# icsharpcode/SharpZipLib

Hardware: NVIDIA B200
Metric: DEFLATE level-6 compress + inflate GB/s (uncompressed) at 1/2/4/8 B200 vs C# ref (higher is better)
Workload: dtype u8

## Files before the change

### include/b200z.h

```cpp
#ifndef B200Z_H
#define B200Z_H
#include <stdint.h>
#ifdef __cplusplus
extern "C" {
#endif

typedef enum b200z_status {
	B200Z_OK = 0,
	B200Z_E_ARG = 1,
	B200Z_E_STATE = 2,
	B200Z_E_DATA = 3,
	B200Z_E_INTERNAL = 4,
	B200Z_E_CUDA = 5,
	B200Z_E_UNSUPPORTED = 6,
	B200Z_E_NOMEM = 7,
	B200Z_E_NEED_INPUT = 8
} b200z_status;

enum { B200Z_WRAP_RAW = 0, B200Z_WRAP_ZLIB = 1, B200Z_WRAP_GZIP = 2, B200Z_WRAP_RAW_CRC32 = 3  };
enum { B200Z_STRATEGY_DEFAULT = 0, B200Z_STRATEGY_FILTERED = 1, B200Z_STRATEGY_HUFFMAN_ONLY = 2 };
enum {
	B200Z_END_FINISH = 0,
	B200Z_END_FLUSH_FINISH = 1,
	B200Z_END_FLUSH = 2
};

const char *b200z_last_error(void);
int b200z_version(void);
int b200z_init(int device);
int b200z_static_tables_size(void);
int b200z_static_tables_export(uint8_t *blob, int32_t cap);
int b200z_static_tables_import(const uint8_t *blob, int32_t len);
int b200z_static_tables_broadcast(void *nccl_comm, int32_t root, int32_t rank, void *cuda_stream);

int b200z_crc32(const uint8_t *buf, int64_t len, uint32_t *value);
int b200z_adler32(const uint8_t *buf, int64_t len, uint32_t *value);
int b200z_checksum_batch_device(int kind, const uint8_t *d_data, const int64_t *off, const int64_t *len, int32_t n,
                                uint32_t *d_value, void *cuda_stream);

typedef struct b200z_plan b200z_plan;

#define B200Z_HIST_NONE 0
#define B200Z_HIST_DICTIONARY 1
#define B200Z_HIST_CONTINUE 2
typedef struct b200z_history {
	int32_t kind;
	int32_t check_seeded;
	const int64_t *hist_len;
	const int64_t *pos_base;
	const int32_t *bit_base;
	const uint8_t *const *hist_mask;
	const int32_t *chunk_count;
	const int64_t *const *chunk_len;
	const int32_t *undrained_last;
	void *const *engine_state;
	struct b200z_stored_state *stored_state;
} b200z_history;
typedef struct b200z_stored_state {
	int32_t strstart, block_start;
	uint32_t slides, input_off;
} b200z_stored_state;
int64_t b200z_engine_state_bytes(void);
int b200z_deflate_plan_create_ex(int32_t n, const int64_t *in_len, int level, int strategy, int wrap, int end_mode,
                                 const b200z_history *hist, b200z_plan **plan);

int b200z_deflate_plan_create(int32_t n, const int64_t *in_len, int level, int strategy, int wrap, int end_mode,
                              b200z_plan **plan);
int b200z_inflate_plan_create(int32_t n, const int64_t *comp_len, const int64_t *out_cap, int wrap, b200z_plan **plan);
int b200z_inflate_plan_create_ex(int32_t n, const int64_t *comp_len, const int64_t *out_cap, int wrap,
                                 const int64_t *dict_len, b200z_plan **plan);
int b200z_inflate_plan_set_start_bits(b200z_plan *plan, const int32_t *start_bit);
int b200z_inflate_plan_set_lengths(b200z_plan *plan, const int64_t *comp_len, const int64_t *dict_len);
int b200z_plan_get_restart_points(b200z_plan *plan, int64_t *bit, int64_t *out_pos, void *cuda_stream);
int b200z_plan_get_stats(b200z_plan *plan, uint32_t *v, int32_t cap, void *cuda_stream);
int b200z_plan_destroy(b200z_plan *plan);
int64_t b200z_plan_in_bytes(const b200z_plan *plan);
int64_t b200z_plan_out_bytes(const b200z_plan *plan);
int64_t b200z_plan_in_offset(const b200z_plan *plan, int32_t i);
int64_t b200z_plan_data_offset(const b200z_plan *plan, int32_t i);
int64_t b200z_plan_out_offset(const b200z_plan *plan, int32_t i);
int64_t b200z_plan_out_capacity(const b200z_plan *plan, int32_t i);
int64_t b200z_plan_workspace_bytes(const b200z_plan *plan);
int32_t b200z_plan_launches(const b200z_plan *plan);
int b200z_plan_set_timing(b200z_plan *plan, int enable);
int b200z_plan_get_timings(b200z_plan *plan, char *names, int32_t names_cap, float *ms, int32_t cap, int32_t *count);
int b200z_plan_run(b200z_plan *plan, const uint8_t *d_in, uint8_t *d_out, int64_t *d_out_len, int32_t *d_status,
                   uint32_t *d_check, int64_t *d_in_used, void *cuda_stream);
#define B200Z_STAGE_SEARCH 1
#define B200Z_STAGE_ENCODE 2
int b200z_plan_run_stages(b200z_plan *plan, const uint8_t *d_in, uint8_t *d_out, int64_t *d_out_len, int32_t *d_status,
                          uint32_t *d_check, int64_t *d_in_used, int stages, void *cuda_stream);

int b200z_plan_pack(b200z_plan *plan, const uint8_t *d_out, const int64_t *d_out_len, uint8_t *d_packed,
                    int64_t *d_packed_off, void *cuda_stream);

typedef struct b200z_pipeline b200z_pipeline;
int b200z_deflate_pipeline_create(int32_t n, const int64_t *in_len, int level, int strategy, int wrap, int end_mode, int depth,
                                  b200z_pipeline **pipe);
int b200z_inflate_pipeline_create(int32_t n, const int64_t *comp_len, const int64_t *out_cap, int wrap, int depth,
                                  b200z_pipeline **pipe);
int b200z_pipeline_submit(b200z_pipeline *pipe, const uint8_t *const *in);
int b200z_pipeline_collect(b200z_pipeline *pipe, uint8_t *const *out, const int64_t *out_cap, int64_t *out_len, int64_t *in_used,
                           uint32_t *check, int32_t *status);
int32_t b200z_pipeline_in_flight(const b200z_pipeline *pipe);
int b200z_pipeline_destroy(b200z_pipeline *pipe);

int b200z_deflate_batch(const uint8_t *const *in, const int64_t *in_len, int32_t n, int level, int strategy, int wrap,
                        int end_mode, uint8_t *const *out, const int64_t *out_cap, int64_t *out_len, uint32_t *check,
                        int32_t *status);
int b200z_inflate_batch(const uint8_t *const *in, const int64_t *in_len, int32_t n, int wrap, uint8_t *const *out,
                        const int64_t *out_cap, int64_t *out_len, int64_t *in_used, uint32_t *check, int32_t *status);
int b200z_release_cached(void);

int b200z_device_count(void);
int b200z_partition_by_bytes(const int64_t *len, int32_t n, int32_t parts, int32_t *first);
int b200z_deflate_batch_multi(const int32_t *devices, int32_t n_devices, const uint8_t *const *in, const int64_t *in_len, int32_t n,
                              int level, int strategy, int wrap, int end_mode, uint8_t *const *out, const int64_t *out_cap,
                              int64_t *out_len, uint32_t *check, int32_t *status);
int b200z_inflate_batch_multi(const int32_t *devices, int32_t n_devices, const uint8_t *const *in, const int64_t *in_len, int32_t n,
                              int wrap, uint8_t *const *out, const int64_t *out_cap, int64_t *out_len, int64_t *in_used,
                              uint32_t *check, int32_t *status);
int64_t b200z_deflate_bound(int64_t len);

int b200z_deflater_create(int level, int raw , void **h);
int b200z_deflater_destroy(void *h);
int b200z_deflater_reset(void *h);
int b200z_deflater_set_level(void *h, int level);
// ... 52 lines not shown
```

### sharpziplib_b200/_lib.py

```python
import ctypes as C
import os

_HERE = os.path.dirname(os.path.abspath(__file__))
SO_PATH = os.path.join(_HERE, "libb200z.so")

OK, E_ARG, E_STATE, E_DATA, E_INTERNAL, E_CUDA, E_UNSUPPORTED, E_NOMEM, E_NEED_INPUT = range(9)
WRAP_RAW, WRAP_ZLIB, WRAP_GZIP, WRAP_RAW_CRC32 = 0, 1, 2, 3
END_FINISH, END_FLUSH_FINISH, END_FLUSH = 0, 1, 2


class SharpZipBaseException(Exception):
    """Mirror of ICSharpCode.SharpZipLib.SharpZipBaseException (Core/Exceptions/SharpZipBaseException.cs)."""


class StreamDecodingException(SharpZipBaseException):
    pass


class B200zUnsupported(NotImplementedError):
    """A call sequence this build does not accelerate (never emulated on the CPU)."""


class B200zCudaError(RuntimeError):
    pass


class InvalidOperationException(RuntimeError):
    pass


def raise_for(rc):
    if rc == OK:
        return
    msg = lib().b200z_last_error().decode("utf-8", "replace")
    code = rc & 0xFF
    if code == E_ARG:
        raise ValueError(msg)
    if code == E_STATE:
        raise InvalidOperationException(msg)
    if code == E_DATA:
        raise SharpZipBaseException(msg)
    if code == E_UNSUPPORTED:
        raise B200zUnsupported(msg)
    if code == E_CUDA:
        raise B200zCudaError(msg)
    if code == E_NOMEM:
        raise MemoryError(msg)
    if code == E_NEED_INPUT:
        raise SharpZipBaseException("Unexpected EOF")
    raise RuntimeError("b200z status %d: %s" % (rc, msg))


_lib = None

_SIGS = {
    "b200z_last_error": (C.c_char_p, []),
    "b200z_version": (C.c_int, []),
    "b200z_init": (C.c_int, [C.c_int]),
    "b200z_static_tables_size": (C.c_int, []),
    "b200z_static_tables_export": (C.c_int, [C.c_void_p, C.c_int32]),
    "b200z_static_tables_import": (C.c_int, [C.c_void_p, C.c_int32]),
    "b200z_crc32": (C.c_int, [C.c_void_p, C.c_int64, C.POINTER(C.c_uint32)]),
    "b200z_adler32": (C.c_int, [C.c_void_p, C.c_int64, C.POINTER(C.c_uint32)]),
    "b200z_checksum_batch_device": (C.c_int, [C.c_int, C.c_void_p, C.c_void_p, C.c_void_p, C.c_int32, C.c_void_p, C.c_void_p]),
    "b200z_deflate_plan_create": (C.c_int, [C.c_int32, C.c_void_p, C.c_int, C.c_int, C.c_int, C.c_int, C.POINTER(C.c_void_p)]),
    "b200z_deflate_plan_create_ex": (C.c_int, [C.c_int32, C.c_void_p, C.c_int, C.c_int, C.c_int, C.c_int, C.c_void_p,
                                               C.POINTER(C.c_void_p)]),
    "b200z_inflate_plan_create": (C.c_int, [C.c_int32, C.c_void_p, C.c_void_p, C.c_int, C.POINTER(C.c_void_p)]),
    "b200z_inflate_plan_create_ex": (C.c_int, [C.c_int32, C.c_void_p, C.c_void_p, C.c_int, C.c_void_p, C.POINTER(C.c_void_p)]),
    "b200z_inflate_plan_set_start_bits": (C.c_int, [C.c_void_p, C.c_void_p]),
    "b200z_plan_get_restart_points": (C.c_int, [C.c_void_p, C.c_void_p, C.c_void_p, C.c_void_p]),
    "b200z_inflate_plan_set_lengths": (C.c_int, [C.c_void_p, C.c_void_p, C.c_void_p]),
    "b200z_plan_get_stats": (C.c_int, [C.c_void_p, C.c_void_p, C.c_int32, C.c_void_p]),
    "b200z_plan_data_offset": (C.c_int64, [C.c_void_p, C.c_int32]),
    "b200z_plan_destroy": (C.c_int, [C.c_void_p]),
    "b200z_plan_in_bytes": (C.c_int64, [C.c_void_p]),
    "b200z_plan_out_bytes": (C.c_int64, [C.c_void_p]),
    "b200z_plan_in_offset": (C.c_int64, [C.c_void_p, C.c_int32]),
    "b200z_plan_out_offset": (C.c_int64, [C.c_void_p, C.c_int32]),
    "b200z_plan_out_capacity": (C.c_int64, [C.c_void_p, C.c_int32]),
    "b200z_plan_workspace_bytes": (C.c_int64, [C.c_void_p]),
    "b200z_plan_launches": (C.c_int32, [C.c_void_p]),
    "b200z_plan_set_timing": (C.c_int, [C.c_void_p, C.c_int]),
    "b200z_plan_get_timings": (C.c_int, [C.c_void_p, C.c_char_p, C.c_int32, C.c_void_p, C.c_int32, C.POINTER(C.c_int32)]),
    "b200z_plan_pack": (C.c_int, [C.c_void_p, C.c_void_p, C.c_void_p, C.c_void_p, C.c_void_p, C.c_void_p]),
    "b200z_plan_run": (C.c_int, [C.c_void_p, C.c_void_p, C.c_void_p, C.c_void_p, C.c_void_p, C.c_void_p, C.c_void_p, C.c_void_p]),
    "b200z_plan_run_stages": (C.c_int, [C.c_void_p, C.c_void_p, C.c_void_p, C.c_void_p, C.c_void_p, C.c_void_p, C.c_void_p, C.c_int,
                                        C.c_void_p]),
    "b200z_deflate_batch": (C.c_int, [C.c_void_p, C.c_void_p, C.c_int32, C.c_int, C.c_int, C.c_int, C.c_int, C.c_void_p, C.c_void_p, C.c_void_p, C.c_void_p, C.c_void_p]),
    "b200z_inflate_batch": (C.c_int, [C.c_void_p, C.c_void_p, C.c_int32, C.c_int, C.c_void_p, C.c_void_p, C.c_void_p, C.c_void_p, C.c_void_p, C.c_void_p]),
    "b200z_release_cached": (C.c_int, []),
    "b200z_device_count": (C.c_int, []),
    "b200z_static_tables_broadcast": (C.c_int, [C.c_void_p, C.c_int32, C.c_int32, C.c_void_p]),
    "b200z_aes_derive_keys": (C.c_int, [C.c_void_p, C.c_void_p, C.c_void_p, C.c_int32, C.c_int32, C.c_void_p]),
    "b200z_aes_state_bytes": (C.c_int64, []),
    "b200z_aes_device": (C.c_int, [C.c_void_p, C.c_void_p, C.c_void_p, C.c_void_p, C.c_int64, C.c_int32, C.c_int32, C.c_void_p, C.c_int32,
                                   C.c_void_p, C.c_int32, C.c_void_p, C.c_void_p]),
    "b200z_aes_batch": (C.c_int, [C.c_void_p, C.c_void_p, C.c_int32, C.c_int32, C.c_void_p, C.c_int32, C.c_void_p, C.c_void_p]),
    "b200z_aes_transform_create": (C.c_int, [C.c_void_p, C.c_int32, C.c_void_p, C.c_int32, C.c_int32, C.POINTER(C.c_void_p)]),
    "b200z_aes_transform_block": (C.c_int, [C.c_void_p, C.c_void_p, C.c_int64, C.c_void_p]),
    "b200z_aes_transform_pwd_verifier": (C.c_int, [C.c_void_p, C.c_void_p]),
    "b200z_aes_transform_auth_code": (C.c_int, [C.c_void_p, C.c_void_p]),
    "b200z_aes_transform_destroy": (C.c_int, [C.c_void_p]),
    "b200z_pkzip_generate_keys": (C.c_int, [C.c_void_p, C.c_int64, C.c_void_p]),
    "b200z_pkzip_device": (C.c_int, [C.c_void_p, C.c_void_p, C.c_void_p, C.c_void_p, C.c_int32, C.c_void_p, C.c_int32, C.c_void_p]),
    "b200z_pkzip_batch": (C.c_int, [C.c_void_p, C.c_void_p, C.c_int32, C.c_void_p, C.c_int32, C.c_void_p]),
    "b200z_partition_by_bytes": (C.c_int, [C.c_void_p, C.c_int32, C.c_int32, C.c_void_p]),
    "b200z_deflate_batch_multi": (C.c_int, [C.c_void_p, C.c_int32, C.c_void_p, C.c_void_p, C.c_int32, C.c_int, C.c_int, C.c_int, C.c_int, C.c_void_p, C.c_void_p, C.c_void_p, C.c_void_p, C.c_void_p]),
    "b200z_inflate_batch_multi": (C.c_int, [C.c_void_p, C.c_int32, C.c_void_p, C.c_void_p, C.c_int32, C.c_int, C.c_void_p, C.c_void_p, C.c_void_p, C.c_void_p, C.c_void_p, C.c_void_p]),
    "b200z_deflate_pipeline_create": (C.c_int, [C.c_int32, C.c_void_p, C.c_int, C.c_int, C.c_int, C.c_int, C.c_int, C.POINTER(C.c_void_p)]),
    "b200z_inflate_pipeline_create": (C.c_int, [C.c_int32, C.c_void_p, C.c_void_p, C.c_int, C.c_int, C.POINTER(C.c_void_p)]),
    "b200z_pipeline_submit": (C.c_int, [C.c_void_p, C.c_void_p]),
    "b200z_pipeline_collect": (C.c_int, [C.c_void_p, C.c_void_p, C.c_void_p, C.c_void_p, C.c_void_p, C.c_void_p, C.c_void_p]),
    "b200z_pipeline_in_flight": (C.c_int32, [C.c_void_p]),
    "b200z_pipeline_destroy": (C.c_int, [C.c_void_p]),
    "b200z_deflate_bound": (C.c_int64, [C.c_int64]),
    "b200z_engine_state_bytes": (C.c_int64, []),
    "b200z_deflater_create": (C.c_int, [C.c_int, C.c_int, C.POINTER(C.c_void_p)]),
    "b200z_deflater_destroy": (C.c_int, [C.c_void_p]),
    "b200z_deflater_reset": (C.c_int, [C.c_void_p]),
    "b200z_deflater_set_level": (C.c_int, [C.c_void_p, C.c_int]),
    "b200z_deflater_get_level": (C.c_int, [C.c_void_p, C.POINTER(C.c_int)]),
    "b200z_deflater_set_strategy": (C.c_int, [C.c_void_p, C.c_int]),
    "b200z_deflater_set_dictionary": (C.c_int, [C.c_void_p, C.c_void_p, C.c_int32]),
    "b200z_deflater_set_input": (C.c_int, [C.c_void_p, C.c_void_p, C.c_int32]),
    "b200z_deflater_flush": (C.c_int, [C.c_void_p]),
# ... 54 lines not shown
```

### sharpziplib_b200/csrc/b200z_api.cu

```cuda
#include <algorithm>
#include <cstdarg>
#include <cstdio>
#include <cstring>
#include <functional>
#include <mutex>
#include <thread>
#include <utility>

#include "b200z_internal.cuh"
#include <dlfcn.h>

namespace b200z {

static thread_local std::string g_err;
static std::mutex g_mu;
static thread_local int t_device = -1;

void set_error(const char *fmt, ...) {
	char buf[512];
	va_list ap;
	va_start(ap, fmt);
	vsnprintf(buf, sizeof(buf), fmt, ap);
	va_end(ap);
	g_err = buf;
// ... 463 lines not shown
	}
	const int n = plan->n;
	std::vector<int64_t> dl((size_t)n);
	std::vector<uint32_t> d32((size_t)n);
	for (int i = 0; i < n; i++) {
		const int64_t D = dict_len ? dict_len[i] : 0;
		if (comp_len[i] < 0 || comp_len[i] > plan->comp_cap[(size_t)i] || D < 0 || D > plan->dict_cap[(size_t)i]) {
			set_error("stream %d: %lld compressed / %lld dictionary bytes exceed what the plan was created for (%lld / %lld)", i,
			          (long long)comp_len[i], (long long)D, (long long)plan->comp_cap[(size_t)i], (long long)plan->dict_cap[(size_t)i]);
			return B200Z_E_ARG;
		}
		dl[(size_t)i] = comp_len[i];
		d32[(size_t)i] = (uint32_t)D;
	}
	for (int i = 0; i < n; i++) {
		if (!plan->hist.empty()) plan->hist[(size_t)i] = d32[(size_t)i];
		plan->in_off[(size_t)i] = plan->comp_off[(size_t)i] - d32[(size_t)i];
		plan->in_len[(size_t)i] = comp_len[i] + d32[(size_t)i];
	}
	if (n) {
		B200Z_CUDA(cudaMemcpy(plan->ws.at<int64_t>(plan->o_in_len), dl.data(), 8ull * n, cudaMemcpyHostToDevice));
		B200Z_CUDA(cudaMemcpy(plan->ws.at<uint32_t>(plan->o_hist), d32.data(), 4ull * n, cudaMemcpyHostToDevice));
	}
	return B200Z_OK;
}

int b200z_plan_get_restart_points(b200z_plan *plan, int64_t *bit, int64_t *out_pos, void *cuda_stream) {
	DeviceGuard guard(plan ? plan->device : -1);
	if (!plan || plan->kind != 1 || (plan->n > 0 && (!bit || !out_pos))) {
		set_error("bad arguments");
		return B200Z_E_ARG;
	}
	if (plan->n == 0) return B200Z_OK;
	std::vector<int64_t> rp(2 * (size_t)plan->n);
	cudaStream_t s = (cudaStream_t)cuda_stream;
	B200Z_CUDA(cudaMemcpyAsync(rp.data(), plan->ws.at<int64_t>(plan->o_restart), 16ull * plan->n, cudaMemcpyDeviceToHost, s));
	B200Z_CUDA(cudaStreamSynchronize(s));
	for (int i = 0; i < plan->n; i++) {
		bit[i] = rp[2 * (size_t)i];
		out_pos[i] = rp[2 * (size_t)i + 1];
	}
	return B200Z_OK;
}

int b200z_plan_get_stats(b200z_plan *plan, uint32_t *v, int32_t cap, void *cuda_stream) {
	DeviceGuard guard(plan ? plan->device : -1);
	if (!plan || plan->kind != 1 || !v || cap < 0) {
		set_error("bad arguments");
		return B200Z_E_ARG;
	}
	return inflate_plan_stats(plan, v, cap, (cudaStream_t)cuda_stream);
}

int b200z_plan_set_timing(b200z_plan *plan, int enable) {
	if (!plan) return B200Z_E_ARG;
	plan->timing = enable != 0;
	plan->ev_used = 0;
	return B200Z_OK;
}

int b200z_plan_get_timings(b200z_plan *plan, char *names, int32_t names_cap, float *ms, int32_t cap, int32_t *count) {
	DeviceGuard guard(plan ? plan->device : -1);
	if (!plan || !ms || !count) return B200Z_E_ARG;
	*count = 0;
	std::string nm;
	for (int i = 0; i + 1 < plan->ev_used && *count < cap; i++) {
		float t = 0;
		cudaError_t e = cudaEventElapsedTime(&t, plan->ev[i], plan->ev[i + 1]);
		if (e != cudaSuccess) return cuda_fail(e, "cudaEventElapsedTime", __FILE__, __LINE__);
		ms[*count] = t;
		nm += plan->ev_name[i];
		nm += ";";
		++*count;
	}
	if (names && names_cap > 0) {
		strncpy(names, nm.c_str(), (size_t)names_cap - 1);
		names[names_cap - 1] = 0;
	}
	return B200Z_OK;
}

int b200z_plan_destroy(b200z_plan *plan) {
	DeviceGuard guard(plan ? plan->device : -1);
	if (!plan) return B200Z_OK;
	for (cudaEvent_t e : plan->ev) cudaEventDestroy(e);
	plan->ws.release();
	delete plan;
	return B200Z_OK;
}
int64_t b200z_plan_in_bytes(const b200z_plan *p) { return p->in_bytes; }
int64_t b200z_plan_out_bytes(const b200z_plan *p) { return p->out_bytes; }
int64_t b200z_plan_in_offset(const b200z_plan *p, int32_t i) { return p->in_off[i]; }
int64_t b200z_plan_data_offset(const b200z_plan *p, int32_t i) {
	return p->in_off[i] + (p->hist.empty() ? 0 : p->hist[i]);
}
int64_t b200z_plan_out_offset(const b200z_plan *p, int32_t i) { return p->out_off[i]; }
int64_t b200z_plan_out_capacity(const b200z_plan *p, int32_t i) { return p->out_cap[i]; }
int64_t b200z_plan_workspace_bytes(const b200z_plan *p) { return p->ws.size; }
int32_t b200z_plan_launches(const b200z_plan *p) { return p->launches; }

int b200z_plan_run(b200z_plan *plan, const uint8_t *d_in, uint8_t *d_out, int64_t *d_out_len, int32_t *d_status,
                   uint32_t *d_check, int64_t *d_in_used, void *cuda_stream) {
	return b200z_plan_run_stages(plan, d_in, d_out, d_out_len, d_status, d_check, d_in_used, B200Z_STAGE_SEARCH | B200Z_STAGE_ENCODE,
	                             cuda_stream);
}

// ... 1328 lines not shown
```

### sharpziplib_b200/csrc/b200z_deflate.cu

```cuda
#include <cuda_pipeline.h>

#include "b200z_internal.cuh"
#include "b200z_tma.cuh"

namespace b200z {

constexpr int kRun = 65536;
constexpr int kTile = 32768;
constexpr int kTileData = 2 * kTile + 320;
constexpr int kMatchThreads = 1024;
constexpr int kMatchClasses = 16;

__device__ __forceinline__ uint32_t same_hash_mask(uint32_t h, bool valid, int lane) {
	uint32_t eq = __ballot_sync(0xffffffffu, valid);
#pragma unroll
	for (int b = 0; b < 15; b++) {
		const bool bit = (h >> b) & 1u;
		const uint32_t bal = __ballot_sync(0xffffffffu, bit);
		eq &= bit ? bal : ~bal;
	}
	return valid ? eq : (1u << lane);
}

constexpr int kLinkChunk = 512;
constexpr int kLinkProducers = 8;
constexpr int kLinkThreads = 32 * (1 + kLinkProducers);
constexpr int kLinkRebase = 16384;
constexpr int kLinksSmem = 65536 + 2 * kLinkChunk * 4;

__global__ void __launch_bounds__(kLinkThreads) k_links(const uint8_t *__restrict__ in, uint16_t *__restrict__ link,
                                                        const int64_t *__restrict__ in_off, const int64_t *__restrict__ in_len,
                                                        const int2 *__restrict__ run_desc, const uint32_t *__restrict__ hist,
                                                        const uint8_t *__restrict__ hmask, const int64_t *__restrict__ hm_off,
                                                        uint32_t run_len) {
	extern __shared__ __align__(16) uint8_t lsm[];
	uint16_t *head = reinterpret_cast<uint16_t *>(lsm);
	uint32_t *info = reinterpret_cast<uint32_t *>(lsm + 65536);
	const int lane = threadIdx.x & 31, warp = threadIdx.x >> 5;
	const int2 rd = run_desc[blockIdx.x];
	const uint32_t n = (uint32_t)in_len[rd.x];
	const uint8_t *data = in + in_off[rd.x];
	uint16_t *lnk = link + in_off[rd.x];
	const uint32_t start = (uint32_t)rd.y;
	const uint32_t run_end = (n - start > run_len) ? start + run_len : n;
	const uint32_t warm = start >= 32768u ? start - 32768u : 0u;
	const uint32_t H = hist[rd.x];
	const uint8_t *hm = hmask + hm_off[rd.x];
	for (int i = threadIdx.x; i < 16384; i += kLinkThreads) reinterpret_cast<uint32_t *>(head)[i] = 0;
	uint32_t winbase = warm;
	auto produce = [&](uint32_t cb, int which) {
		constexpr int G = kLinkChunk / 32 / kLinkProducers;
		uint32_t hh[G];
		bool vv[G];
#pragma unroll
		for (int j = 0; j < G; j++) {
			const uint32_t p = cb + 32u * (uint32_t)(warp - 1 + kLinkProducers * j) + lane;
			bool valid = p + 2 < n;
			uint32_t h = 0;
			if (p + 2 < n) h = hash3(__ldg(data + p), __ldg(data + p + 1), __ldg(data + p + 2));
			if (p < H && valid) valid = __ldg(hm + p) == 0;
			hh[j] = h;
			vv[j] = valid;
		}
#pragma unroll
// ... 39 lines not shown
				const uint32_t v = head[h];
				const bool valid = (w >> 15) & 1u;
				uint32_t q = v ? winbase + v - 1 : 0xFFFFFFFFu;
				if ((w >> 16) & 1u) q = base + ((w >> 17) & 31u);
				__syncwarp();
				if (valid && ((w >> 22) & 1u)) head[h] = (uint16_t)(p - winbase + 1);
				__syncwarp();
				const uint32_t d = (valid && q != 0xFFFFFFFFu) ? p - q : 0u;
				if (p >= start && p < run_end) lnk[p] = (d <= (uint32_t)kMaxDist) ? (uint16_t)d : (uint16_t)0;
				w = wn;
			}
		} else if (cb + kLinkChunk < run_end) {
			produce(cb + kLinkChunk, which ^ 1);
		}
		__syncthreads();
	}
}

__global__ void __launch_bounds__(kMatchThreads, 1)
    k_match(const uint8_t *__restrict__ in, const uint16_t *__restrict__ link, uint2 *__restrict__ mt,
            const int64_t *__restrict__ in_off, const int64_t *__restrict__ in_len, const int2 *__restrict__ tile_desc,
            const uint32_t *__restrict__ hist, const int64_t *__restrict__ bias, uint32_t *__restrict__ scratch, LevelParams lp) {
	extern __shared__ __align__(16) uint8_t smem[];
	uint8_t *s_data = smem;
	uint16_t *s_link = reinterpret_cast<uint16_t *>(smem + kTileData);
	const int2 td = tile_desc[blockIdx.x];
	const uint32_t n = (uint32_t)in_len[td.x];
	const int64_t off = in_off[td.x];
	const uint8_t *data = in + off;
	const uint16_t *lnk = link + off;
	const uint32_t t0 = (uint32_t)td.y;
	const uint32_t t1 = (n - t0 > (uint32_t)kTile) ? t0 + kTile : n;
	const uint32_t w0 = t0 >= (uint32_t)kTile ? t0 - kTile : 0u;
	uint32_t dend = t1 + 272;
	if (dend > n) dend = n;
	__shared__ BulkBarrier s_bar;
	if (threadIdx.x == 0) bulk_barrier_init(&s_bar);
	__syncthreads();
	{
		const uint32_t nbytes = dend - w0;
		const uint32_t nvec = nbytes >> 4;
		const uint32_t nl = t1 - w0;
		const uint32_t nlv = nl >> 3;
		if (threadIdx.x == 0) {
			bulk_expect(&s_bar, 16u * (nvec + nlv));
			bulk_copy_start(&s_bar, s_data, data + w0, 16u * nvec);
			bulk_copy_start(&s_bar, s_link, lnk + w0, 16u * nlv);
		}
		for (uint32_t i = (nvec << 4) + threadIdx.x; i < nbytes; i += kMatchThreads) s_data[i] = data[w0 + i];
		for (uint32_t i = (nlv << 3) + threadIdx.x; i < nl; i += kMatchThreads) s_link[i] = lnk[w0 + i];
	}
	bulk_wait(&s_bar, 0);
	__syncthreads();
	uint2 *out = mt + off;
	const uint32_t chain = (uint32_t)lp.chain, budgetB = chain >> 2;
	const uint32_t H = hist[td.x];
	const uint32_t ab = (uint32_t)bias[td.x];
	__shared__ uint32_t s_cls[2][kMatchClasses];
	if (threadIdx.x < 2 * kMatchClasses) (&s_cls[0][0])[threadIdx.x] = 0;
	__syncthreads();
	uint16_t *order = reinterpret_cast<uint16_t *>(scratch + off + t0);
	uint32_t cw[4] = {0u, 0u, 0u, 0u};
	const int lane = threadIdx.x & 31;
#pragma unroll
	for (int k = 0; k < kTile / kMatchThreads; k++) {
		const uint32_t p = t0 + threadIdx.x + (uint32_t)k * kMatchThreads;
		uint32_t cls = 0;
		if (p < t1 && p >= H) {
			const uint32_t la = n - p;
			uint32_t d = la >= (uint32_t)kMinMatch ? (uint32_t)s_link[p - w0] : 0u;
			if (d > (uint32_t)kMaxDist - (is_slide_pos(p + ab) ? 1u : 0u)) d = 0;
			if (d == 0) out[p] = make_uint2(0u, 0u);
			else {
				const uint32_t is = p - w0;
				uint32_t dist = d, hops = 1;
				while (hops < 8) {
					const uint32_t l2 = s_link[is - dist];
					if (l2 == 0 || dist + l2 >= (uint32_t)kMaxDist) break;
					dist += l2;
					++hops;
				}
				if (hops < 8) cls = hops <= 1 ? 1u : hops <= 2 ? 2u : hops <= 4 ? 3u : hops <= 6 ? 4u : 5u;
				else {
					uint32_t est = (8u * (uint32_t)kMaxDist) / dist;
					if (est > chain) est = chain;
					cls = est <= 11 ? 6u : est <= 16 ? 7u : est <= 23 ? 8u : est <= 32 ? 9u : est <= 45 ? 10u : est <= 64 ? 11u
					      : est <= 91 ? 12u : est <= 128 ? 13u : est <= 512 ? 14u : 15u;
				}
			}
		}
		const uint32_t peers = __match_any_sync(0xffffffffu, cls);
		if (cls && lane == __ffs((int)peers) - 1) atomicAdd(&s_cls[0][cls], (uint32_t)__popc(peers));
		cw[k >> 3] |= cls << ((k & 7) * 4);
	}
	__syncthreads();
	uint32_t total = 0;
	{
		uint32_t b = 0;
		uint32_t mine = 0;
		for (int c = kMatchClasses - 1; c >= 1; c--) {
			if ((int)threadIdx.x == c) mine = b;
			b += s_cls[0][c];
		}
		total = b;
		__syncthreads();
		if (threadIdx.x >= 1 && threadIdx.x < kMatchClasses) s_cls[1][threadIdx.x] = mine;
		__syncthreads();
	}
#pragma unroll
	for (int k = 0; k < kTile / kMatchThreads; k++) {
		const uint32_t cls = (cw[k >> 3] >> ((k & 7) * 4)) & 15u;
		const uint32_t peers = __match_any_sync(0xffffffffu, cls);
		uint32_t slot = 0;
		const int leader = __ffs((int)peers) - 1;
		if (cls && lane == leader) slot = atomicAdd(&s_cls[1][cls], (uint32_t)__popc(peers));
		slot = __shfl_sync(0xffffffffu, slot, leader);
		if (cls) order[slot + (uint32_t)__popc(peers & ((1u << lane) - 1u))] = (uint16_t)(threadIdx.x + (uint32_t)k * kMatchThreads);
	}
	__syncthreads();
	for (uint32_t i = threadIdx.x; i < total; i += kMatchThreads) {
		const uint32_t p = t0 + (uint32_t)__ldcg(&order[i]);
		uint32_t resA = 0, resB = 0;
		const uint32_t la = n - p;
		const uint32_t d = (uint32_t)s_link[p - w0];
		if (d != 0) {
			const uint32_t maxlen = la < (uint32_t)kMaxMatch ? la : (uint32_t)kMaxMatch;
			const uint32_t nice = la < (uint32_t)lp.nice ? la : (uint32_t)lp.nice;
			const uint32_t is = p - w0;
			const uint8_t *sp = s_data + is;
			uint32_t m = kMinMatch - 1, bd = 0, dist = d, cnt = 0;
			bool haveB = false;
			uint32_t stop = budgetB ? budgetB : chain;
			const uint32_t s0 = sp[0], s1 = sp[1];
			uint32_t scan_end1 = s1, scan_end = sp[2];
			uint32_t sw0, sw1;
			{
				const uint32_t as = is + 2;
				const uint32_t *ws = reinterpret_cast<const uint32_t *>(s_data + (as & ~3u));
				const uint32_t w1 = ws[1], sh = (as & 3u) * 8u;
				sw0 = __funnelshift_r(ws[0], w1, sh);
				sw1 = __funnelshift_r(w1, ws[2], sh);
			}
			for (;;) {
				const uint32_t ic = is - dist;
				const uint8_t *c = s_data + ic;
				++cnt;
				if (c[m] == scan_end && c[m - 1] == scan_end1 && c[0] == s0 && c[1] == s1) {
					uint32_t l = 2;
					if (maxlen >= 10) {
						const uint32_t ac = ic + 2;
						const uint32_t *wc = reinterpret_cast<const uint32_t *>(s_data + (ac & ~3u));
						const uint32_t w1 = wc[1], sh = (ac & 3u) * 8u;
						uint32_t x = __funnelshift_r(wc[0], w1, sh) ^ sw0;
						if (x) {
							l = 2 + ((uint32_t)(__ffs((int)x) - 1) >> 3);
							goto lcp_done;
						}
						x = __funnelshift_r(w1, wc[2], sh) ^ sw1;
						if (x) {
							l = 6 + ((uint32_t)(__ffs((int)x) - 1) >> 3);
							goto lcp_done;
						}
						l = 10;
					}
					while (l + 4 <= maxlen) {
						const uint32_t ac = ic + l, as = is + l;
						const uint32_t *wc = reinterpret_cast<const uint32_t *>(s_data + (ac & ~3u));
						const uint32_t *ws = reinterpret_cast<const uint32_t *>(s_data + (as & ~3u));
						const uint32_t x = __funnelshift_r(wc[0], wc[1], (ac & 3u) * 8u) ^ __funnelshift_r(ws[0], ws[1], (as & 3u) * 8u);
						if (x) {
							l += (uint32_t)(__ffs((int)x) - 1) >> 3;
							goto lcp_done;
						}
						l += 4;
					}
					while (l < maxlen && c[l] == sp[l]) ++l;
				lcp_done:
					if (l > m) {
						m = l;
						bd = dist;
						if (m >= nice) break;
						scan_end1 = sp[m - 1];
						scan_end = sp[m];
					}
				}
				if (cnt == stop) {
					if (stop == chain) break;
					resB = m >= (uint32_t)kMinMatch ? pack_match(m, bd) : 0u;
					haveB = true;
					stop = chain;
				}
				const uint32_t l2 = s_link[is - dist];
				if (l2 == 0) break;
				dist += l2;
				if (dist >= (uint32_t)kMaxDist) break;
			}
			resA = m >= (uint32_t)kMinMatch ? pack_match(m, bd) : 0u;
			if (!haveB) resB = resA;
		}
		out[p] = make_uint2(resA, resB);
	}
}

constexpr int kSegShift = 5;
constexpr int kSeg = 1 << kSegShift;
constexpr int kRound = 32 * kSeg;
constexpr int kParseWarm = 128;
constexpr int kSegStride = kSeg + 2;
constexpr int kParseDatOff = 32 * kSegStride * 8;
constexpr int kParseSmem = kParseDatOff + kRound + 48;

struct ChunkDesc {
	int32_t stream;
	uint32_t c0, c1;
};

__device__ __forceinline__ ParseCarry shfl_carry(const ParseCarry &c, int src) {
	ParseCarry r;
	r.st.p = __shfl_sync(0xffffffffu, c.st.p, src);
	r.st.mlen = __shfl_sync(0xffffffffu, c.st.mlen, src);
	r.st.mstart = __shfl_sync(0xffffffffu, c.st.mstart, src);
	r.st.prevAvail = __shfl_sync(0xffffffffu, c.st.prevAvail, src);
	r.last_top = __shfl_sync(0xffffffffu, c.last_top, src);
	return r;
}

__device__ __forceinline__ ParseCarry clean_carry(uint32_t p) {
	ParseCarry c;
	parse_init(c.st);
	c.st.p = p;
	c.last_top = p;
	return c;
}

struct RoundRec {
	uint32_t p, mlen, mstart, prevAvail, last_top, cnt;
};
__device__ __forceinline__ ParseCarry rec_carry(const RoundRec &r) {
	ParseCarry c;
	c.st.p = r.p;
	c.st.mlen = r.mlen;
	c.st.mstart = r.mstart;
	c.st.prevAvail = r.prevAvail;
	c.last_top = r.last_top;
	return c;
}

__device__ __forceinline__ uint32_t parse_round(uint8_t *smem, const uint8_t *data, const uint16_t *lnk, const uint2 *tab,
                                                uint32_t n, uint32_t H, uint32_t ab, uint32_t base, const LevelParams &lp,
                                                int strategy, ParseCarry &carry, uint32_t *sround) {
	uint2 *s_tab = reinterpret_cast<uint2 *>(smem);
	uint8_t *s_dat = smem + kParseDatOff;
	const int lane = threadIdx.x & 31;
// ... 1252 lines not shown
		    p->fast_head_smem ? nullptr : ws.at<uint16_t>(p->o_fhead), ws.at<uint32_t>(p->o_fcounter));
	} else {
		if (do_search) {
		p->mark(s, "k_links");
		if (p->n_runs) k_links<<<p->n_runs, kLinkThreads, kLinksSmem, s>>>(d_in, link, in_off, in_len, ws.at<int2>(p->o_run_desc), hist,
			                                                         ws.at<uint8_t>(p->o_hmask), ws.at<int64_t>(p->o_hm_off), (uint32_t)p->link_run);
		p->mark(s, "k_match");
		if (p->n_tiles)
			k_match<<<p->n_tiles, kMatchThreads, kTileData + 2 * 2 * kTile, s>>>(d_in, link, mt, in_off, in_len,
			                                                                   ws.at<int2>(p->o_tile_desc), hist, bias, sym, lp);
		}
		if (!do_encode) {
			B200Z_CUDA(cudaGetLastError());
			return B200Z_OK;
		}
		p->mark(s, "k_parse");
		{
			uint32_t *sym_local = ws.at<uint32_t>(p->o_sym_local);
			const uint32_t *rnd_off = ws.at<uint32_t>(p->o_rnd_off);
			RoundRec *recs = ws.at<RoundRec>(p->o_recs);
			uint32_t *rnd_symoff = ws.at<uint32_t>(p->o_rnd_symoff);
			if (p->n_chunks)
				k_parse_chunk<<<p->n_chunks, 32, kParseSmem, s>>>(d_in, link, mt, sym_local, in_off, in_len, ws.at<ChunkDesc>(p->o_chunks),
				                                                 rnd_off, recs, ws.at<RoundRec>(p->o_ents), hist, bias, lp, p->strategy, parse_warm());
			k_parse_fix<<<n, 32, kParseSmem, s>>>(d_in, link, mt, sym_local, in_off, in_len, rnd_off, recs, ws.at<RoundRec>(p->o_ents),
			                                      p->parse_chunk, hist, bias, lp, p->strategy);
			k_parse_scan<<<n, 256, 0, s>>>(d_in, in_off, in_len, rnd_off, recs, rnd_symoff, sym, nsyms, nblocks, blk_off, blk_start,
			                               blk_ptop, hist, p->end_mode);
			if (p->n_rgroups)
				k_parse_gather<<<p->n_rgroups, 128, 0, s>>>(sym_local, sym, in_off, in_len, ws.at<int2>(p->o_rgroups), rnd_off, recs,
				                                           rnd_symoff, blk_off, blk_start, blk_ptop, hist);
		}
	}
	p->mark(s, "k_plan");
	k_plan<<<p->n_blkmax, kPlanThreads, 0, s>>>(sym, in_off, in_len, nsyms, nblocks, blk_off, blk_desc, blk_start, blk_ptop, meta,
	                                   tables, bias, p->end_mode);
	p->mark(s, "k_scan");
	k_scan<<<(n + 127) / 128, 128, 0, s>>>(n, nblocks, blk_off, meta, d_out, out_off, out_cap, d_out_len, d_status,
	                                       d_out_bits, bit_base, p->end_mode);
	p->mark(s, "k_emit");
	k_emit<<<p->n_blkmax, 256, 0, s>>>(d_in, sym, d_out, in_off, out_off, nblocks, blk_off, blk_desc, meta, tables);
	p->mark(s, "checksum");
	if (p->wrap != B200Z_WRAP_RAW && d_check) {
		int rc = checksum_launch(p->wrap == B200Z_WRAP_ZLIB ? 1 : 0, d_in, ws.at<int64_t>(p->o_ck_off), ws.at<int64_t>(p->o_ck_len), n,
		                         ws.at<CkTile>(p->o_ck_desc), p->n_ck_tiles, ws.at<unsigned long long>(p->o_ck_acc), d_check,
		                         ck_fresh, s);
		if (rc) return rc;
	}
	p->mark(s, "end");
	B200Z_CUDA(cudaGetLastError());
	return B200Z_OK;
}

}
```

### sharpziplib_b200/csrc/b200z_internal.cuh

```cuda
#pragma once
#include <cuda_runtime.h>
#include <stdint.h>
#include <string>
#include <vector>

#include "../../include/b200z.h"
#include "b200z_core.cuh"
#include "b200z_crc.cuh"

namespace b200z {

void set_error(const char *fmt, ...);
int cuda_fail(cudaError_t e, const char *what, const char *file, int line);

#define B200Z_CUDA(call)                                                                   \
	do {                                                                                   \
		cudaError_t e__ = (call);                                                          \
		if (e__ != cudaSuccess) return ::b200z::cuda_fail(e__, #call, __FILE__, __LINE__); \
	} while (0)

int ensure_init();
int current_device();

struct DeviceGuard {
// ... 72 lines not shown
	int64_t o_in_off = 0, o_in_len = 0, o_out_off = 0, o_out_cap = 0;
	int64_t o_run_desc = 0, o_tile_desc = 0, o_blk_desc = 0, o_blk_off = 0;
	int64_t o_link = 0, o_mt = 0, o_sym = 0, o_nsyms = 0, o_nblocks = 0;
	int64_t o_blk_start = 0, o_blk_ptop = 0, o_meta = 0, o_tables = 0;
	int n_runs = 0, n_tiles = 0, n_blkmax = 0;
	int64_t o_sym_local = 0, o_chunks = 0, o_rgroups = 0, o_rnd_off = 0, o_recs = 0, o_ents = 0, o_rnd_symoff = 0;
	int n_chunks = 0, n_rgroups = 0;
	uint32_t parse_chunk = 32768;
	int link_run = 65536;
	int fast_prev_entries = 32768;
	int fast_ctas = 1;
	bool fast_head_smem = false;
	int64_t o_stored = 0, o_slens = 0;
	std::vector<std::vector<uint32_t>> sched_cum;
	std::vector<int32_t> undrained;
	std::vector<void *> engine_state;
	struct b200z_stored_state *stored_state = nullptr;
	int64_t o_sched = 0, o_sched_off = 0, o_undrained = 0, o_fstate = 0, o_fhead = 0, o_fcounter = 0;
	int n_stored = 0;
	int64_t o_tok = 0, o_ntok = 0, o_tok_off = 0;
	int64_t o_start_bit = 0, o_pre = 0;
	int64_t o_restart = 0;
	bool has_start_bits = false;
	std::vector<int64_t> comp_off, comp_cap, dict_cap;
	bool inf_parallel = true;
	int64_t o_win_base = 0, o_win_stream = 0, o_cand = 0, o_ftiles = 0, o_fs_list = 0, o_ctr = 0, o_segs = 0, o_seg_list = 0;
	int64_t o_rounds = 0, o_hdrs = 0, o_mlist = 0, o_mt_off = 0, o_match_cap = 0, o_str_nm = 0, o_fallback = 0;
	uint32_t nwin_total = 0, n_ftiles = 0, fs_cap = 0, round_cap = 0, hdr_cap = 0;
	int dec1_grid = 0, dec2_grid = 0, find3_grid = 0;
	int64_t o_ck_desc = 0, o_ck_acc = 0;
	int n_ck_tiles = 0;
	bool timing = false;
	std::vector<cudaEvent_t> ev;
	std::vector<const char *> ev_name;
	int ev_used = 0;
	void mark(cudaStream_t s, const char *next_name) {
		if (!timing) return;
		if ((int)ev.size() <= ev_used) {
			cudaEvent_t e;
			cudaEventCreate(&e);
			ev.push_back(e);
			ev_name.push_back("");
		}
		cudaEventRecord(ev[ev_used], s);
		ev_name[ev_used] = next_name;
		++ev_used;
	}
};

namespace b200z {
int deflate_plan_build(b200z_plan *p);
int deflate_plan_run(b200z_plan *p, const uint8_t *d_in, uint8_t *d_out, int64_t *d_out_len, int32_t *d_status,
                     uint32_t *d_check, int64_t *d_out_bits, cudaStream_t s, int stages);
int inflate_plan_build(b200z_plan *p);
int inflate_plan_stats(b200z_plan *p, uint32_t *v, int32_t cap, cudaStream_t s);
int inflate_plan_run(b200z_plan *p, const uint8_t *d_in, uint8_t *d_out, int64_t *d_out_len, int32_t *d_status,
                     uint32_t *d_check, int64_t *d_in_used, cudaStream_t s);
int checksum_launch(int kind, const uint8_t *d_data, const int64_t *d_off, const int64_t *d_len, int32_t n,
                    const CkTile *d_tiles, int32_t n_tiles, unsigned long long *d_acc, uint32_t *d_value, int fresh,
                    cudaStream_t s);
int checksum_tiles(const int64_t *len, int32_t n, std::vector<CkTile> &tiles, int kind, bool dynamic = false);
int checksum_init_tables();
}
```

Before: 16.23.

## Rewrite hash-chain walk with sentinel links and absolute index stepping

Rewrites zero link entries in shared memory to a 0xFFFF sentinel so the chain walk needs no zero-link test, since a sentinel hop always moves past the maximum distance. The match-finder inner loop now steps absolute candidate indices (byte offsets into the link array and the scan-end position) instead of recomputing them from a distance. It also prefetches the next link before comparing, and splits the two chain budgets into nested loops. A debug export entry point for the link and match tables is added as well. The intent is fewer instructions and dependent loads per chain hop, at the cost of an extra shared-memory pass over the link array per tile.

```diff
diff --git a/include/b200z.h b/include/b200z.h
--- a/include/b200z.h
+++ b/include/b200z.h
@@ -73,6 +73,7 @@
 int b200z_inflate_plan_set_lengths(b200z_plan *plan, const int64_t *comp_len, const int64_t *dict_len);
 int b200z_plan_get_restart_points(b200z_plan *plan, int64_t *bit, int64_t *out_pos, void *cuda_stream);
 int b200z_plan_get_stats(b200z_plan *plan, uint32_t *v, int32_t cap, void *cuda_stream);
+int b200z_plan_get_match_table(b200z_plan *plan, int32_t i, uint16_t *link, uint32_t *ab, void *cuda_stream);
 int b200z_plan_destroy(b200z_plan *plan);
 int64_t b200z_plan_in_bytes(const b200z_plan *plan);
 int64_t b200z_plan_out_bytes(const b200z_plan *plan);
diff --git a/sharpziplib_b200/_lib.py b/sharpziplib_b200/_lib.py
--- a/sharpziplib_b200/_lib.py
+++ b/sharpziplib_b200/_lib.py
@@ -72,6 +72,7 @@
     "b200z_plan_get_restart_points": (C.c_int, [C.c_void_p, C.c_void_p, C.c_void_p, C.c_void_p]),
     "b200z_inflate_plan_set_lengths": (C.c_int, [C.c_void_p, C.c_void_p, C.c_void_p]),
     "b200z_plan_get_stats": (C.c_int, [C.c_void_p, C.c_void_p, C.c_int32, C.c_void_p]),
+    "b200z_plan_get_match_table": (C.c_int, [C.c_void_p, C.c_int32, C.c_void_p, C.c_void_p, C.c_void_p]),
     "b200z_plan_data_offset": (C.c_int64, [C.c_void_p, C.c_int32]),
     "b200z_plan_destroy": (C.c_int, [C.c_void_p]),
     "b200z_plan_in_bytes": (C.c_int64, [C.c_void_p]),
diff --git a/sharpziplib_b200/csrc/b200z_api.cu b/sharpziplib_b200/csrc/b200z_api.cu
--- a/sharpziplib_b200/csrc/b200z_api.cu
+++ b/sharpziplib_b200/csrc/b200z_api.cu
@@ -539,6 +539,15 @@
 	return inflate_plan_stats(plan, v, cap, (cudaStream_t)cuda_stream);
 }
 
+int b200z_plan_get_match_table(b200z_plan *plan, int32_t i, uint16_t *link, uint32_t *ab, void *cuda_stream) {
+	DeviceGuard guard(plan ? plan->device : -1);
+	if (!plan || plan->kind != 0 || plan->level < 5 || i < 0 || i >= plan->n || !ab) {
+		set_error("bad arguments");
+		return B200Z_E_ARG;
+	}
+	return deflate_plan_match_table(plan, i, link, ab, (cudaStream_t)cuda_stream);
+}
+
 int b200z_plan_set_timing(b200z_plan *plan, int enable) {
 	if (!plan) return B200Z_E_ARG;
 	plan->timing = enable != 0;
diff --git a/sharpziplib_b200/csrc/b200z_deflate.cu b/sharpziplib_b200/csrc/b200z_deflate.cu
--- a/sharpziplib_b200/csrc/b200z_deflate.cu
+++ b/sharpziplib_b200/csrc/b200z_deflate.cu
@@ -10,6 +10,7 @@
 constexpr int kTileData = 2 * kTile + 320;
 constexpr int kMatchThreads = 1024;
 constexpr int kMatchClasses = 16;
+constexpr uint32_t kNoLink = 0xFFFFu;
 
 __device__ __forceinline__ uint32_t same_hash_mask(uint32_t h, bool valid, int lane) {
 	uint32_t eq = __ballot_sync(0xffffffffu, valid);
@@ -155,13 +156,17 @@
 	}
 	bulk_wait(&s_bar, 0);
 	__syncthreads();
+	for (uint32_t i = threadIdx.x; i < (t1 - w0 + 1) / 2; i += kMatchThreads) {
+		const uint32_t v = reinterpret_cast<uint32_t *>(s_link)[i];
+		reinterpret_cast<uint32_t *>(s_link)[i] = v | ((v & 0xFFFFu) ? 0u : kNoLink) | ((v >> 16) ? 0u : kNoLink << 16);
+	}
+	__shared__ uint32_t s_cls[2][kMatchClasses];
+	if (threadIdx.x < 2 * kMatchClasses) (&s_cls[0][0])[threadIdx.x] = 0;
+	__syncthreads();
 	uint2 *out = mt + off;
 	const uint32_t chain = (uint32_t)lp.chain, budgetB = chain >> 2;
 	const uint32_t H = hist[td.x];
 	const uint32_t ab = (uint32_t)bias[td.x];
-	__shared__ uint32_t s_cls[2][kMatchClasses];
-	if (threadIdx.x < 2 * kMatchClasses) (&s_cls[0][0])[threadIdx.x] = 0;
-	__syncthreads();
 	uint16_t *order = reinterpret_cast<uint16_t *>(scratch + off + t0);
 	uint32_t cw[4] = {0u, 0u, 0u, 0u};
 	const int lane = threadIdx.x & 31;
@@ -171,15 +176,14 @@
 		uint32_t cls = 0;
 		if (p < t1 && p >= H) {
 			const uint32_t la = n - p;
-			uint32_t d = la >= (uint32_t)kMinMatch ? (uint32_t)s_link[p - w0] : 0u;
-			if (d > (uint32_t)kMaxDist - (is_slide_pos(p + ab) ? 1u : 0u)) d = 0;
-			if (d == 0) out[p] = make_uint2(0u, 0u);
+			const uint32_t d = la >= (uint32_t)kMinMatch ? (uint32_t)s_link[p - w0] : kNoLink;
+			if (d > (uint32_t)kMaxDist - (is_slide_pos(p + ab) ? 1u : 0u)) out[p] = make_uint2(0u, 0u);
 			else {
 				const uint32_t is = p - w0;
 				uint32_t dist = d, hops = 1;
 				while (hops < 8) {
 					const uint32_t l2 = s_link[is - dist];
-					if (l2 == 0 || dist + l2 >= (uint32_t)kMaxDist) break;
+					if (dist + l2 >= (uint32_t)kMaxDist) break;
 					dist += l2;
 					++hops;
 				}
@@ -221,87 +225,90 @@
 		if (cls) order[slot + (uint32_t)__popc(peers & ((1u << lane) - 1u))] = (uint16_t)(threadIdx.x + (uint32_t)k * kMatchThreads);
 	}
 	__syncthreads();
+	const uint8_t *lb = reinterpret_cast<const uint8_t *>(s_link);
 	for (uint32_t i = threadIdx.x; i < total; i += kMatchThreads) {
 		const uint32_t p = t0 + (uint32_t)__ldcg(&order[i]);
-		uint32_t resA = 0, resB = 0;
 		const uint32_t la = n - p;
-		const uint32_t d = (uint32_t)s_link[p - w0];
-		if (d != 0) {
-			const uint32_t maxlen = la < (uint32_t)kMaxMatch ? la : (uint32_t)kMaxMatch;
-			const uint32_t nice = la < (uint32_t)lp.nice ? la : (uint32_t)lp.nice;
-			const uint32_t is = p - w0;
-			const uint8_t *sp = s_data + is;
-			uint32_t m = kMinMatch - 1, bd = 0, dist = d, cnt = 0;
-			bool haveB = false;
-			uint32_t stop = budgetB ? budgetB : chain;
-			const uint32_t s0 = sp[0], s1 = sp[1];
-			uint32_t scan_end1 = s1, scan_end = sp[2];
-			uint32_t sw0, sw1;
-			{
-				const uint32_t as = is + 2;
-				const uint32_t *ws = reinterpret_cast<const uint32_t *>(s_data + (as & ~3u));
-				const uint32_t w1 = ws[1], sh = (as & 3u) * 8u;
-				sw0 = __funnelshift_r(ws[0], w1, sh);
-				sw1 = __funnelshift_r(w1, ws[2], sh);
-			}
+		const uint32_t maxlen = la < (uint32_t)kMaxMatch ? la : (uint32_t)kMaxMatch;
+		const uint32_t nice = la < (uint32_t)lp.nice ? la : (uint32_t)lp.nice;
+		const uint32_t is = p - w0;
+		const uint8_t *sp = s_data + is;
+		const int ic0 = (int)is - (int)s_link[is];
+		int icm = ic0 + (kMinMatch - 1), il = 2 * ic0;
+		const int ilmin = 2 * ((int)is - kMaxDist);
+		uint32_t m = kMinMatch - 1, bd = 0, resB = 0;
+		bool haveB = false;
+		uint32_t left = budgetB ? budgetB : chain, rest = chain - left;
+		const uint32_t s0 = sp[0], s1 = sp[1];
+		uint32_t scan_end1 = s1, scan_end = sp[2];
+		uint32_t sw0, sw1;
+		{
+			const uint32_t as = is + 2;
+			const uint32_t *ws = reinterpret_cast<const uint32_t *>(s_data + (as & ~3u));
+			const uint32_t w1 = ws[1], sh = (as & 3u) * 8u;
+			sw0 = __funnelshift_r(ws[0], w1, sh);
+			sw1 = __funnelshift_r(w1, ws[2], sh);
+		}
+		for (;;) {
 			for (;;) {
-				const uint32_t ic = is - dist;
-				const uint8_t *c = s_data + ic;
-				++cnt;
-				if (c[m] == scan_end && c[m - 1] == scan_end1 && c[0] == s0 && c[1] == s1) {
-					uint32_t l = 2;
-					if (maxlen >= 10) {
-						const uint32_t ac = ic + 2;
-						const uint32_t *wc = reinterpret_cast<const uint32_t *>(s_data + (ac & ~3u));
-						const uint32_t w1 = wc[1], sh = (ac & 3u) * 8u;
-						uint32_t x = __funnelshift_r(wc[0], w1, sh) ^ sw0;
-						if (x) {
-							l = 2 + ((uint32_t)(__ffs((int)x) - 1) >> 3);
-							goto lcp_done;
+				const uint32_t l2 = *reinterpret_cast<const uint16_t *>(lb + il);
+				if (s_data[icm] == scan_end && s_data[icm - 1] == scan_end1) {
+					const uint32_t ic = (uint32_t)(il >> 1);
+					const uint8_t *c = s_data + ic;
+					if (c[0] == s0 && c[1] == s1) {
+						uint32_t l = 2;
+						if (maxlen >= 10) {
+							const uint32_t ac = ic + 2;
+							const uint32_t *wc = reinterpret_cast<const uint32_t *>(s_data + (ac & ~3u));
+							const uint32_t w1 = wc[1], sh = (ac & 3u) * 8u;
+							uint32_t x = __funnelshift_r(wc[0], w1, sh) ^ sw0;
+							if (x) {
+								l = 2 + ((uint32_t)(__ffs((int)x) - 1) >> 3);
+								goto lcp_done;
+							}
+							x = __funnelshift_r(w1, wc[2], sh) ^ sw1;
+							if (x) {
+								l = 6 + ((uint32_t)(__ffs((int)x) - 1) >> 3);
+								goto lcp_done;
+							}
+							l = 10;
 						}
-						x = __funnelshift_r(w1, wc[2], sh) ^ sw1;
-						if (x) {
-							l = 6 + ((uint32_t)(__ffs((int)x) - 1) >> 3);
-							goto lcp_done;
+						while (l + 4 <= maxlen) {
+							const uint32_t ac = ic + l, as = is + l;
+							const uint32_t *wc = reinterpret_cast<const uint32_t *>(s_data + (ac & ~3u));
+							const uint32_t *ws = reinterpret_cast<const uint32_t *>(s_data + (as & ~3u));
+							const uint32_t x = __funnelshift_r(wc[0], wc[1], (ac & 3u) * 8u) ^ __funnelshift_r(ws[0], ws[1], (as & 3u) * 8u);
+							if (x) {
+								l += (uint32_t)(__ffs((int)x) - 1) >> 3;
+								goto lcp_done;
+							}
+							l += 4;
 						}
-						l = 10;
-					}
-					while (l + 4 <= maxlen) {
-						const uint32_t ac = ic + l, as = is + l;
-						const uint32_t *wc = reinterpret_cast<const uint32_t *>(s_data + (ac & ~3u));
-						const uint32_t *ws = reinterpret_cast<const uint32_t *>(s_data + (as & ~3u));
-						const uint32_t x = __funnelshift_r(wc[0], wc[1], (ac & 3u) * 8u) ^ __funnelshift_r(ws[0], ws[1], (as & 3u) * 8u);
-						if (x) {
-							l += (uint32_t)(__ffs((int)x) - 1) >> 3;
-							goto lcp_done;
+						while (l < maxlen && c[l] == sp[l]) ++l;
+					lcp_done:
+						if (l > m) {
+							m = l;
+							bd = is - ic;
+							if (m >= nice) goto walk_done;
+							scan_end1 = sp[m - 1];
+							scan_end = sp[m];
+							icm = (int)(ic + m);
 						}
-						l += 4;
-					}
-					while (l < maxlen && c[l] == sp[l]) ++l;
-				lcp_done:
-					if (l > m) {
-						m = l;
-						bd = dist;
-						if (m >= nice) break;
-						scan_end1 = sp[m - 1];
-						scan_end = sp[m];
 					}
 				}
-				if (cnt == stop) {
-					if (stop == chain) break;
-					resB = m >= (uint32_t)kMinMatch ? pack_match(m, bd) : 0u;
-					haveB = true;
-					stop = chain;
-				}
-				const uint32_t l2 = s_link[is - dist];
-				if (l2 == 0) break;
-				dist += l2;
-				if (dist >= (uint32_t)kMaxDist) break;
-			}
-			resA = m >= (uint32_t)kMinMatch ? pack_match(m, bd) : 0u;
-			if (!haveB) resB = resA;
-		}
-		out[p] = make_uint2(resA, resB);
+				icm -= (int)l2;
+				il -= 2 * (int)l2;
+				if ((il <= ilmin) | (--left == 0)) break;
+			}
+			if (il <= ilmin || rest == 0) break;
+			resB = m >= (uint32_t)kMinMatch ? pack_match(m, bd) : 0u;
+			haveB = true;
+			left = rest;
+			rest = 0;
+		}
+	walk_done:
+		const uint32_t resA = m >= (uint32_t)kMinMatch ? pack_match(m, bd) : 0u;
+		out[p] = make_uint2(resA, haveB ? resB : resA);
 	}
 }
 
@@ -1660,4 +1667,12 @@
 	return B200Z_OK;
 }
 
-}
+int deflate_plan_match_table(b200z_plan *p, int32_t i, uint16_t *link, uint32_t *ab, cudaStream_t s) {
+	const int64_t off = p->in_off[i], n = p->in_len[i], H = p->hist.empty() ? 0 : p->hist[i];
+	if (link) B200Z_CUDA(cudaMemcpyAsync(link, p->ws.at<uint16_t>(p->o_link) + off, 2 * n, cudaMemcpyDeviceToHost, s));
+	B200Z_CUDA(cudaMemcpyAsync(ab, p->ws.at<uint2>(p->o_mt) + off + H, 8 * (n - H), cudaMemcpyDeviceToHost, s));
+	B200Z_CUDA(cudaStreamSynchronize(s));
+	return B200Z_OK;
+}
+
+}
diff --git a/sharpziplib_b200/csrc/b200z_internal.cuh b/sharpziplib_b200/csrc/b200z_internal.cuh
--- a/sharpziplib_b200/csrc/b200z_internal.cuh
+++ b/sharpziplib_b200/csrc/b200z_internal.cuh
@@ -148,6 +148,7 @@
 int deflate_plan_build(b200z_plan *p);
 int deflate_plan_run(b200z_plan *p, const uint8_t *d_in, uint8_t *d_out, int64_t *d_out_len, int32_t *d_status,
                      uint32_t *d_check, int64_t *d_out_bits, cudaStream_t s, int stages);
+int deflate_plan_match_table(b200z_plan *p, int32_t i, uint16_t *link, uint32_t *ab, cudaStream_t s);
 int inflate_plan_build(b200z_plan *p);
 int inflate_plan_stats(b200z_plan *p, uint32_t *v, int32_t cap, cudaStream_t s);
 int inflate_plan_run(b200z_plan *p, const uint8_t *d_in, uint8_t *d_out, int64_t *d_out_len, int32_t *d_status,
```

After: 17.83 (median of 6 runs). 1.1x the previous value.
